# HilaManor/AudioEditingCode

Measured on AMD Instinct MI355X. Metric: edited-clips/sec (200-step inv+edit, 10 s@16 kHz), higher is better.
Workload: dtype f32

## Files before the change

audioeditingcode_amd/_lib.py:

```python
import ctypes
import os

import torch

_HERE = os.path.dirname(os.path.abspath(__file__))
LIB_PATH = os.path.join(_HERE, "libaed.so")


class aed_op(ctypes.Structure):
    _fields_ = [("code", ctypes.c_int32), ("flags", ctypes.c_int32), ("i", ctypes.c_int32 * 40),
                ("f", ctypes.c_float * 8), ("p", ctypes.c_void_p * 10)]


OP_NOP, OP_CONV_GEMM, OP_GN_STATS, OP_GN_APPLY, OP_LAYERNORM, OP_ATTENTION, OP_GEGLU, OP_COPY2D, \
    OP_TIME_EMBED, OP_SOFTMAX_ROWS, OP_TRANSPOSE, OP_AXPBY, OP_INVERT_STEP, OP_REVERSE_STEP, OP_DDIM_STEP, \
    OP_ADVANCE, OP_REFLECT_PAD, OP_MAGNITUDE, OP_NCHW_TO_NHWC, OP_NHWC_TO_NCHW, OP_SPLITK_REDUCE, \
    OP_GN_SCALE_SHIFT, OP_GN_SMALL, OP_XATTN_FOLD, OP_ROTARY, OP_SNAKE, OP_SA_STEP, OP_GAUSS_SAMPLE, \
    OP_REVERSE_STEP_VARIANTS, OP_DRIFT_STEP_VARIANTS, OP_REVERSE_STEP_ROWS = range(31)
OP_NAMES = ["nop", "conv_gemm", "gn_stats", "gn_apply", "layernorm", "attention", "geglu", "copy2d", "time_embed",
            "softmax_rows", "transpose", "axpby", "invert_step", "reverse_step", "ddim_step", "advance",
            "reflect_pad", "magnitude", "nchw_to_nhwc", "nhwc_to_nchw", "splitk_reduce", "gn_scale_shift", "gn_small",
            "xattn_fold", "rotary", "snake", "sa_step", "gauss_sample", "reverse_step_variants",
            "drift_step_variants", "reverse_step_rows"]
OP_PC_PROBE, OP_PC_JACOBIAN, OP_PC_ORTHONORMALISE = 31, 32, 33
# ... 3 lines not shown
T5_ATTN_HEAD_SIZES = (8, 16, 32, 64)
T5_ATTN_MAX_L = 512
OP_LAYERNORM_ROWS, OP_ADD_ROWS, OP_GELU_NEW, OP_CAUSAL_ATTENTION = 41, 42, 43, 44
LM_ATTN_HEAD_SIZES = (8, 16, 32, 64)
LM_ATTN_MAX_NK = 1024
SEG_MAX_P = 8
PC_TAB_STRIDE = 4
PC_MAX_EV = 8
ACT_NONE, ACT_SILU, ACT_LEAKY, ACT_TANH, ACT_LOGCLAMP = range(5)
COEF_STRIDE = 8
SA_COEF_STRIDE = 12

_lib = None


class AedError(RuntimeError):
    pass


def lib():
    global _lib
    if _lib is None:
        if not os.path.exists(LIB_PATH):
            raise AedError(f"{LIB_PATH} is missing: build it with `python __graft_entry__.py` "
                           f"(audioeditingcode_amd/csrc/build.sh). There is no CPU fallback.")
        L = ctypes.CDLL(LIB_PATH)
        vp, ci, cf = ctypes.c_void_p, ctypes.c_int, ctypes.c_float
        L.aed_version.restype = ci
        L.aed_last_error.restype = ctypes.c_char_p
        L.aed_device_info.argtypes = [ctypes.POINTER(ci), ctypes.POINTER(ci), ctypes.c_char_p, ci]
        L.aed_launch.argtypes = [ctypes.POINTER(aed_op), vp]
        L.aed_tape_run.argtypes = [ctypes.POINTER(aed_op), ci, vp]
        L.aed_tape_profile.argtypes = [ctypes.POINTER(aed_op), ci, vp, ctypes.POINTER(cf)]
        L.aed_graph_begin.argtypes = [vp]
        L.aed_graph_end.argtypes = [vp, ctypes.POINTER(vp)]
        L.aed_graph_launch.argtypes = [vp, vp]
        L.aed_graph_destroy.argtypes = [vp]
        L.aed_stream_create_cu_mask.argtypes = [ctypes.POINTER(vp), ctypes.POINTER(ctypes.c_uint32), ci, ci]
        L.aed_stream_destroy.argtypes = [vp]
        L.aed_cu_census.argtypes = [vp, ci, ci, vp]
        u64 = ctypes.c_uint64
        L.aed_image_load.argtypes = [ctypes.c_char_p, ci, ctypes.POINTER(vp)]
        L.aed_image_free.argtypes = [vp]
        L.aed_image_run.argtypes = [vp, ctypes.c_char_p, vp]
        L.aed_image_program.argtypes = [vp, ctypes.c_char_p, ctypes.POINTER(ctypes.POINTER(aed_op)), ctypes.POINTER(ci)]
        L.aed_image_buffer.argtypes = [vp, ctypes.c_char_p, ctypes.POINTER(vp), ctypes.POINTER(u64)]
        L.aed_image_copy_in.argtypes = [vp, ctypes.c_char_p, vp, u64, vp]
        L.aed_image_copy_out.argtypes = [vp, ctypes.c_char_p, vp, u64, vp]
        L.aed_event_create.argtypes = [ctypes.POINTER(vp)]
        L.aed_event_record.argtypes = [vp, vp]
        L.aed_event_elapsed_ms.argtypes = [vp, vp, ctypes.POINTER(cf)]
        L.aed_event_destroy.argtypes = [vp]
        fp = ctypes.POINTER(cf)
        L.aed_get_zs_from_xts.argtypes = [vp, vp, vp, vp, vp, cf, ci, fp, ci, ci, vp, vp, ctypes.c_int64, vp]
        L.aed_reverse_step_with_custom_noise.argtypes = [vp, vp, vp, vp, cf, ci, fp, ci, vp, vp, ctypes.c_int64, vp]
        L.aed_reverse_step_variants.argtypes = [vp, vp, vp, ci, fp, ci, vp, vp, ctypes.c_int64, vp]
        L.aed_reverse_step_clips.argtypes = [vp, vp, vp, ci, fp, ci, vp, vp, ctypes.c_int64, vp]
        L.aed_reverse_step_rows.argtypes = [vp, vp, vp, ci, fp, ci, ctypes.POINTER(vp), vp, ctypes.c_int64, vp]
        L.aed_drift_step_variants.argtypes = [vp, vp, vp, ci, fp, ci, vp, vp, vp, ci, ci, vp, vp, ci, cf, ctypes.c_int64, vp]
        L.aed_sample_xts_from_x0.argtypes = [vp, vp, vp, vp, vp, ci, ctypes.c_int64, vp]
        L.aed_mx_quantize_rows.argtypes = [vp, vp, vp, ctypes.c_longlong, ci, vp]
        L.aed_resample_sinc.argtypes = [vp, ci, ctypes.c_int64, vp, ci, ci, ci, vp, ctypes.c_int64, vp]
        L.aed_sa_get_zs_from_xts.argtypes = [vp, vp, vp, vp, cf, fp, vp, ci, vp, vp, ctypes.c_int64, vp]
        L.aed_sa_reverse_step_with_custom_noise.argtypes = [vp, vp, vp, cf, fp, vp, vp, vp, ctypes.c_int64, vp]
        L.aed_sa_reverse_step_variants.argtypes = [vp, vp, vp, ci, fp, ctypes.POINTER(ci), ci, vp, vp, vp, ctypes.c_int64, vp]
        for name in ("aed_launch", "aed_tape_run", "aed_tape_profile", "aed_graph_begin", "aed_graph_end",
                     "aed_graph_launch", "aed_graph_destroy", "aed_stream_create_cu_mask", "aed_stream_destroy",
                     "aed_cu_census", "aed_image_load", "aed_image_free", "aed_image_run", "aed_image_program",
                     "aed_image_buffer", "aed_image_copy_in", "aed_image_copy_out", "aed_event_create", "aed_event_record", "aed_event_elapsed_ms", "aed_event_destroy", "aed_get_zs_from_xts",
                     "aed_reverse_step_with_custom_noise", "aed_reverse_step_variants", "aed_reverse_step_clips", "aed_reverse_step_rows", "aed_drift_step_variants", "aed_sample_xts_from_x0", "aed_device_info",
                     "aed_sa_get_zs_from_xts", "aed_sa_reverse_step_with_custom_noise", "aed_sa_reverse_step_variants",
                     "aed_mx_quantize_rows", "aed_resample_sinc"):
            getattr(L, name).restype = ci
        if L.aed_version() != 4:
            raise AedError("libaed.so ABI version mismatch")
        _lib = L
    return _lib


EXPORTS = ["aed_version", "aed_last_error", "aed_device_info", "aed_launch", "aed_tape_run", "aed_tape_profile",
           "aed_graph_begin", "aed_graph_end", "aed_graph_launch", "aed_graph_destroy", "aed_stream_create_cu_mask",
           "aed_stream_destroy", "aed_cu_census", "aed_image_load", "aed_image_free", "aed_image_run", "aed_image_program",
           "aed_image_buffer", "aed_image_copy_in", "aed_image_copy_out", "aed_event_create",
           "aed_event_record", "aed_event_elapsed_ms", "aed_event_destroy", "aed_get_zs_from_xts",
           "aed_reverse_step_with_custom_noise", "aed_reverse_step_variants", "aed_reverse_step_clips", "aed_reverse_step_rows", "aed_drift_step_variants", "aed_sample_xts_from_x0",
           "aed_sa_get_zs_from_xts",
           "aed_sa_reverse_step_with_custom_noise", "aed_sa_reverse_step_variants", "aed_mx_quantize_rows", "aed_resample_sinc"]


def check(rc, what=""):
    if rc != 0:
        raise AedError(f"{what} failed (rc={rc}): {lib().aed_last_error().decode()}")


def current_stream_ptr():
    import torch
    return ctypes.c_void_p(torch.cuda.current_stream().cuda_stream)
```

audioeditingcode_amd/csrc/api.hip:

```cpp
#include <stdarg.h>
#include <string.h>
#include <vector>
#include "aed_common.h"

static thread_local char g_err[512] = "";
void aed_set_error(const char* fmt, ...) {
    va_list ap;
    va_start(ap, fmt);
    vsnprintf(g_err, sizeof(g_err), fmt, ap);
    va_end(ap);
}

static int g_cus = 0;
int aed_num_cus() {
    if (g_cus == 0) {
        int dev = 0;
        hipDeviceProp_t prop;
        if (hipGetDevice(&dev) == hipSuccess && hipGetDeviceProperties(&prop, dev) == hipSuccess)
            g_cus = prop.multiProcessorCount;
        if (g_cus <= 0) g_cus = 256;
    }
    return g_cus;
}

__global__ void cu_census_kernel(uint32_t* out, int spin) {
    long long t0 = __builtin_readcyclecounter();
    while (__builtin_readcyclecounter() - t0 < spin) __builtin_amdgcn_s_sleep(8);
    if (threadIdx.x == 0) {
        out[2 * blockIdx.x] = __builtin_amdgcn_s_getreg((4) | (0 << 6) | (31 << 11));
        out[2 * blockIdx.x + 1] = __builtin_amdgcn_s_getreg((20) | (0 << 6) | (31 << 11));
    }
}

typedef int (*launcher_t)(const aed_op*, hipStream_t);
static int launch_nop(const aed_op*, hipStream_t) { return 0; }
static int launch_retired(const aed_op* op, hipStream_t) {
    aed_set_error("opcode %d was retired in ABI v4 (fused into conv_gemm: ln_mode / geglu slots)", op->code);
    return 3;
}
int launch_conv_gemm_x6(const aed_op* op, hipStream_t s);
int launch_conv_gemm_f8(const aed_op* op, hipStream_t s);
static int launch_conv_gemm_any(const aed_op* op, hipStream_t s) {
    if (op->flags & 64) return launch_conv_gemm_f8(op, s);
    return (op->flags & 4) ? launch_conv_gemm_x6(op, s) : launch_conv_gemm(op, s);
}
static launcher_t g_table[AED_OP_COUNT] = {
    launch_nop,
    launch_conv_gemm_any,
    launch_gn_stats, launch_gn_apply, launch_retired, launch_attention, launch_retired, launch_copy2d,
    launch_time_embed, launch_softmax_rows, launch_transpose, launch_axpby, launch_invert_step,
    launch_reverse_step, launch_ddim_step, launch_advance, launch_reflect_pad, launch_magnitude,
    launch_layout, launch_layout, launch_splitk_reduce, launch_gn_scale_shift, launch_gn_small, launch_xattn_fold,
    launch_rotary, launch_snake, launch_sa_step, launch_gauss_sample, launch_reverse_step_variants,
    launch_drift_step_variants, launch_reverse_step_rows, launch_pc_probe, launch_pc_jacobian, launch_pc_orthonormalise,
    launch_sa_step_variants, launch_reverse_step_segments,
    launch_t5_embed, launch_rmsnorm, launch_t5_attention, launch_gated_act,
    nullptr,
    launch_layernorm_rows, launch_add_rows, launch_gelu_new, launch_causal_attention,
};

extern "C" {

int aed_version(void) { return AED_VERSION; }
const char* aed_last_error(void) { return g_err; }

int aed_device_info(int* cu_count, int* lds_bytes, char* arch, int arch_len) {
    int dev = 0;
    hipDeviceProp_t prop;
    AED_CHECK_HIP(hipGetDevice(&dev));
    AED_CHECK_HIP(hipGetDeviceProperties(&prop, dev));
    if (cu_count) *cu_count = prop.multiProcessorCount;
    if (lds_bytes) *lds_bytes = (int)prop.maxSharedMemoryPerMultiProcessor;
    if (arch && arch_len > 0) {
        strncpy(arch, prop.gcnArchName, arch_len - 1);
        arch[arch_len - 1] = 0;
    }
    return 0;
}

int aed_launch(const aed_op* op, void* stream) {
    AED_REQUIRE(op != nullptr, "aed_launch: null op");
    AED_REQUIRE(op->code >= 0 && op->code < AED_OP_COUNT && g_table[op->code] != nullptr, "aed_launch: bad opcode %d", op->code);
    return g_table[op->code](op, (hipStream_t)stream);
}

int aed_tape_run(const aed_op* ops, int n, void* stream) {
    AED_REQUIRE(ops != nullptr || n == 0, "aed_tape_run: null tape");
    for (int k = 0; k < n; ++k) {
        const aed_op* op = ops + k;
        if (op->code < 0 || op->code >= AED_OP_COUNT || g_table[op->code] == nullptr) {
            aed_set_error("aed_tape_run: bad opcode %d at op %d", op->code, k);
            return 2;
        }
        int rc = g_table[op->code](op, (hipStream_t)stream);
        if (rc) {
            char tmp[400];
            strncpy(tmp, g_err, sizeof(tmp) - 1);
            tmp[sizeof(tmp) - 1] = 0;
            aed_set_error("op %d (code %d): %s", k, op->code, tmp);
            return rc;
        }
    }
    return 0;
}

int aed_tape_profile(const aed_op* ops, int n, void* stream, float* ms_host) {
    AED_REQUIRE(ops && ms_host, "aed_tape_profile: null argument");
    std::vector<hipEvent_t> ev(n + 1);
    for (int k = 0; k <= n; ++k) AED_CHECK_HIP(hipEventCreate(&ev[k]));
    AED_CHECK_HIP(hipEventRecord(ev[0], (hipStream_t)stream));
    for (int k = 0; k < n; ++k) {
        int rc = aed_launch(ops + k, stream);
        if (rc) return rc;
        AED_CHECK_HIP(hipEventRecord(ev[k + 1], (hipStream_t)stream));
    }
    AED_CHECK_HIP(hipEventSynchronize(ev[n]));
    for (int k = 0; k < n; ++k) AED_CHECK_HIP(hipEventElapsedTime(&ms_host[k], ev[k], ev[k + 1]));
    for (int k = 0; k <= n; ++k) (void)hipEventDestroy(ev[k]);
    return 0;
}

int aed_graph_begin(void* stream) {
    AED_CHECK_HIP(hipStreamBeginCapture((hipStream_t)stream, hipStreamCaptureModeThreadLocal));
    return 0;
}
int aed_graph_end(void* stream, void** graph_exec_out) {
    hipGraph_t graph = nullptr;
    AED_CHECK_HIP(hipStreamEndCapture((hipStream_t)stream, &graph));
    hipGraphExec_t exec = nullptr;
    hipError_t e = hipGraphInstantiate(&exec, graph, nullptr, nullptr, 0);
    (void)hipGraphDestroy(graph);
    if (e != hipSuccess) {
        aed_set_error("hipGraphInstantiate: %s", hipGetErrorString(e));
        return 1;
    }
    *graph_exec_out = (void*)exec;
// ... 60 lines not shown
```

audioeditingcode_amd/csrc/cg_params.h:

```cpp
#pragma once
#include "aed_common.h"

typedef float f32x16 __attribute__((ext_vector_type(16)));

struct CGParams {
    const float* A;
    const float* W;
    const float* bias;
    float* C;
    const float* res;
    const float* rowvec;
    float* ws;
    long long* dbg;
    const float* A2;
    int diag;
    int gm;
    int M, N, K;
    int lda, ldc, ldr, ld_rv;
    int IH, IW, OH, OW, Cin;
    int KH, KW, stride, pad_h, pad_w, dil_h, dil_w, up;
    int a_bs;
    int vIH, vIW;
    int o_mul, o_add, o_len, out_bs;
    int in_act, out_act, accumulate, ksplit;
// ... 11 lines not shown
    const float* kbias;
    int geglu;
    const unsigned char* Wq;
    const unsigned char* Wsc;
};

__device__ __forceinline__ float in_transform(float v, int act, float slope) {
    if (act == AED_ACT_SILU) return v / (1.0f + __expf(-v));
    if (act == AED_ACT_LEAKY) return v > 0.0f ? v : v * slope;
    return v;
}

__device__ __forceinline__ float gelu_exact(float g) { return 0.5f * g * (1.0f + erff(g * 0.70710678118654752440f)); }
__device__ __forceinline__ float glu_gate(float g, int kind) { return kind == 2 ? g / (1.0f + expf(-g)) : gelu_exact(g); }

__device__ __forceinline__ void store_out(const CGParams& p, int m, int n, float v) {
    int b = m / p.rpb;
    int q = m - b * p.rpb;
    int o = q * p.o_mul + p.o_add;
    if ((unsigned)o >= (unsigned)p.o_len) return;
    size_t row = (size_t)b * p.out_bs + o;
    if (p.bias) v += p.bias[n];
    if (p.rowvec && !p.ln_mode) v += p.rowvec[(size_t)b * p.ld_rv + n];
    if (p.res) v += p.res[row * p.ldr + n];
    v = aed_apply_act(v, p.out_act, p.out_p);
    float* dst = p.C + row * p.ldc + n;
    if (p.accumulate == 1) v += *dst;
    else if (p.accumulate == 2) v = (*dst + v) / p.out_div;
    *dst = v;
}

int cg_fill_params(const aed_op* op, CGParams& p, int bkt);
int launch_lin_gemm(const CGParams& p, int cfg, hipStream_t s);
```

audioeditingcode_amd/csrc/conv_gemm.hip:

```cpp
#include "cg_params.h"

template <int BM, int BN, int WROWS, int WCOLS, bool GENERIC, int DEPTH, int BKT, bool PLAIN>
__global__ __launch_bounds__(256, (BM * BN >= 128 * 128) ? 2 : 1) void conv_gemm_kernel(CGParams p) {
    constexpr int WM = BM / WROWS, WN = BN / WCOLS;
    constexpr int TM = WM / 32, TN = WN / 32;
    constexpr int LDS_LD = BKT + 4;
    constexpr int STAGE = (BM + BN) * LDS_LD;
    constexpr int TPR = BKT / 4;
    constexpr int RPP = 256 / TPR;
    constexpr int PA = BM / RPP, PB = BN / RPP;
    constexpr int NKB = BKT / 8;
    static_assert(WROWS * WCOLS == 4, "4 waves");
    static_assert(TM >= 1 && TN >= 1 && PA >= 1 && PB >= 1, "tile");

    __shared__ __attribute__((aligned(16))) float lds[2 * STAGE];

    const int tid = threadIdx.x;
    const int lane = tid & 63;
    const int wave = tid >> 6;
    const int wr = wave / WCOLS, wc = wave % WCOLS;
    int tile_x = blockIdx.x, tile_y = blockIdx.y;
    if (gridDim.z == 1) {
        const unsigned nx = gridDim.x, nwg = nx * gridDim.y;
        const unsigned orig = blockIdx.y * nx + blockIdx.x;
// ... 356 lines not shown
                "conv_gemm: operand exceeds the 32-bit element-offset range");
    if (p.ksplit < 1) p.ksplit = 1;
    if (p.ksplit > p.nchunks) p.ksplit = p.nchunks;
    if (p.ksplit > 1) AED_REQUIRE(p.ws != nullptr, "conv_gemm: split-K needs a workspace");
    if (p.ln_mode)
        AED_REQUIRE(p.ksplit == 1 && p.KH * p.KW == 1 && p.rowvec && p.bias && p.in_act == 0,
                    "conv_gemm: fused LayerNorm needs a 1-tap, unsplit GEMM with folded weights");
    if (p.C1 > 0)
        AED_REQUIRE(p.A2 && p.C1 % 64 == 0 && p.C1 < p.Cin && p.lda2 % 4 == 0 && ((uintptr_t)p.A2 % 16) == 0 &&
                        (long long)(p.M / p.rpb) * p.a_bs2 + (long long)p.IH * p.IW * p.lda2 < (1LL << 31),
                    "conv_gemm: bad two-source split C1=%d of Cin=%d", p.C1, p.Cin);
    if (p.geglu)
        AED_REQUIRE(p.ksplit == 1 && p.N % 64 == 0 && !p.res && p.out_act == 0 && p.accumulate == 0 && p.o_mul == 1 &&
                        p.o_add == 0 && p.o_len >= p.rpb && (p.ln_mode || !p.rowvec),
                    "conv_gemm: the GEGLU epilogue needs an unsplit GEMM with packed N %% 64 == 0 and a plain epilogue");
    return 0;
}

template <int BM, int BN, int WR, int WC, int DEPTH, int BKT>
static void launch_cfg(const CGParams& p, bool plain, hipStream_t s) {
    dim3 grid(aed_cdiv(p.N, BN), aed_cdiv(p.M, BM), p.ksplit);
    if (plain)
        hipLaunchKernelGGL((conv_gemm_kernel<BM, BN, WR, WC, false, DEPTH, BKT, true>), grid, dim3(256), 0, s, p);
    else
        hipLaunchKernelGGL((conv_gemm_kernel<BM, BN, WR, WC, false, DEPTH, BKT, false>), grid, dim3(256), 0, s, p);
}

template <int BM, int BN, int WR, int WC>
static void launch_generic(const CGParams& p, hipStream_t s) {
    dim3 grid(aed_cdiv(p.N, BN), aed_cdiv(p.M, BM), p.ksplit);
    hipLaunchKernelGGL((conv_gemm_kernel<BM, BN, WR, WC, true, 1, 32, false>), grid, dim3(256), 0, s, p);
}

int launch_conv_gemm(const aed_op* op, hipStream_t s) {
    CGParams p;
    const int32_t* i = op->i;
    const int Cin = i[11];
    const bool generic = (Cin % 32 != 0) || (i[3] % 4 != 0) || ((uintptr_t)op->p[0] % 16 != 0) ||
                         ((uintptr_t)op->p[1] % 16 != 0);
    int cfg = i[29];
    if (cfg >= 10) {
        int rc = cg_fill_params(op, p, 32);
        if (rc) return rc;
        return launch_lin_gemm(p, cfg, s);
    }
    if (cfg == 0) {
        const int cus = aed_num_cus();
        const int M = i[0], N = i[1], ks = i[28] > 1 ? i[28] : 1;
        auto blocks = [&](int bm, int bn) { return (long)aed_cdiv(M, bm) * aed_cdiv(N, bn) * ks; };
        if (N <= 32) cfg = 5;
        else if (M <= 32) cfg = 6;
        else if (blocks(128, 128) >= (long)cus && N >= 128) cfg = 1;
        else if (blocks(128, 64) >= 2L * cus && N >= 64) cfg = 2;
        else cfg = 4;
        if (N < 64 && cfg != 5) cfg = 5;
    }
    if (generic && (cfg == 1 || cfg == 2 || cfg == 3)) cfg = 4;
    const bool bk64 = !generic && (Cin % 64 == 0) && i[30] != 1 && cfg == 4;
    int rc = cg_fill_params(op, p, bk64 ? 64 : 32);
    if (rc) return rc;
    const bool plain = p.in_act == 0 && p.ln_mode == 0;
    AED_REQUIRE(p.sm_group == 0 && p.w_bs == 0 && p.vec_bs == 0 && p.vec_ld == 1,
                "conv_gemm: per-batch weights / grouped softmax exist only in the lin_gemm kernels (tile >= 10)");
    if (p.geglu) AED_REQUIRE(cfg == 1 || cfg == 3, "conv_gemm: the GEGLU epilogue needs 64-wide wave tiles: 128x128 or 64x128 (cfg %d)", cfg);
    if (p.C1 > 0) AED_REQUIRE(!generic, "conv_gemm: two-source A needs the vector path of a tiled kernel");
    switch (cfg) {
        case 1: launch_cfg<128, 128, 2, 2, 2, 32>(p, plain, s); break;
        case 2: launch_cfg<128, 64, 2, 2, 2, 32>(p, plain, s); break;
        case 3: launch_cfg<64, 128, 2, 2, 2, 32>(p, plain, s); break;
        case 4:
            if (generic) launch_generic<64, 64, 2, 2>(p, s);
            else if (bk64) launch_cfg<64, 64, 2, 2, 2, 64>(p, plain, s);
            else launch_cfg<64, 64, 2, 2, 3, 32>(p, plain, s);
            break;
        case 5:
            if (generic) launch_generic<128, 32, 4, 1>(p, s);
            else launch_cfg<128, 32, 4, 1, 3, 32>(p, plain, s);
            break;
        case 6:
            if (generic) launch_generic<32, 128, 1, 4>(p, s);
            else launch_cfg<32, 128, 1, 4, 3, 32>(p, plain, s);
            break;
        default: AED_REQUIRE(false, "conv_gemm: bad tile cfg %d", cfg);
    }
    AED_CHECK_HIP(hipGetLastError());
    if (p.ksplit > 1) {
        size_t total = (size_t)p.M * p.N;
        int grid = (int)((((p.N & 3) == 0 ? total >> 2 : total) + 255) / 256);
        if (grid > 2048) grid = 2048;
        hipLaunchKernelGGL(splitk_reduce_kernel, dim3(grid), dim3(256), 0, s, p);
        AED_CHECK_HIP(hipGetLastError());
    }
    return 0;
}

int launch_splitk_reduce_slices(const aed_op* op, int slices, hipStream_t s) {
    CGParams p;
    int rc = cg_fill_params(op, p, 32);
    if (rc) return rc;
    if (slices > 0) p.ksplit = slices;
    size_t total = (size_t)p.M * p.N;
    int grid = (int)((((p.N & 3) == 0 ? total >> 2 : total) + 255) / 256);
    if (grid > 2048) grid = 2048;
    hipLaunchKernelGGL(splitk_reduce_kernel, dim3(grid), dim3(256), 0, s, p);
    AED_CHECK_HIP(hipGetLastError());
    return 0;
}

int launch_splitk_reduce(const aed_op* op, hipStream_t s) { return launch_splitk_reduce_slices(op, 0, s); }
```

audioeditingcode_amd/csrc/conv_gemm_x6.hip:

```cpp
#include "cg_params.h"

typedef __bf16 bf16x8 __attribute__((ext_vector_type(8)));
typedef __bf16 bf16x2 __attribute__((ext_vector_type(2)));
typedef float f32x2 __attribute__((ext_vector_type(2)));

int launch_conv_gemm_x6(const aed_op* op, hipStream_t s);

constexpr int X6_BK = 16;

__device__ __forceinline__ void x6_split_pair(float x0, float x1, unsigned& h, unsigned& m, unsigned& l) {
    h = __builtin_bit_cast(unsigned, __builtin_convertvector((f32x2){x0, x1}, bf16x2));
    float r0 = x0 - __uint_as_float(h << 16);
    float r1 = x1 - __uint_as_float(h & 0xffff0000u);
    asm volatile("" : "+v"(r0), "+v"(r1));
    m = __builtin_bit_cast(unsigned, __builtin_convertvector((f32x2){r0, r1}, bf16x2));
    float q0 = r0 - __uint_as_float(m << 16);
    float q1 = r1 - __uint_as_float(m & 0xffff0000u);
    asm volatile("" : "+v"(q0), "+v"(q1));
    l = __builtin_bit_cast(unsigned, __builtin_convertvector((f32x2){q0, q1}, bf16x2));
}

typedef unsigned u32x4 __attribute__((ext_vector_type(4)));
constexpr unsigned X6_OOB = 0x80000000u;

// ... 253 lines not shown
            if constexpr (KB == 2) {
                bf16x8 af2[TM][3], bw2[TN][3];
                load_frags(lds + cur * STAGE, 1, af2, bw2);
                do_mfmas(af2, bw2);
            }
            hints();
            __syncthreads();
            cur ^= 1;
        }
    }

    float* ln_stat = reinterpret_cast<float*>(lds);
#include "cg_epilogue.h"
}

template <int BM, int BN, int WR, int WC, int DEPTH, bool DIAG, int BK = X6_BK>
static int x6_launch(const CGParams& p, bool plain, int sched, int terms, hipStream_t s) {
    dim3 grid(aed_cdiv(p.N, BN), aed_cdiv(p.M, BM), p.ksplit);
    dim3 block(64 * WR * WC);
#define X6_GO(PL, SC, NT_) hipLaunchKernelGGL((conv_gemm_x6_kernel<BM, BN, WR, WC, DEPTH, PL, SC, NT_, BK>), grid, block, 0, s, p)
    if (terms == 3) {
        if constexpr (DIAG) {
            if (plain) { X6_GO(true, 1, 3); return 0; }
        }
        AED_REQUIRE(false, "conv_gemm_x6: the three-term diagnostic exists for tiles 1 and 8 with a plain A operand");
    }
    if (!plain) X6_GO(false, 1, 6);
    else if (sched) X6_GO(true, 1, 6);
    else X6_GO(true, 0, 6);
#undef X6_GO
    return 0;
}

int launch_conv_gemm_x6(const aed_op* op, hipStream_t s) {
    const int32_t* i = op->i;
    const int Cin = i[11];
    int cfg = i[29];
    const long long batch = i[0] / (i[9] * i[10] > 0 ? i[9] * i[10] : 1);
    const bool fits = (Cin % X6_BK == 0) && (i[3] % 4 == 0) && ((uintptr_t)op->p[0] % 16 == 0) &&
                      ((uintptr_t)op->p[1] % 16 == 0) && cfg < 10 && cfg != 5 && cfg != 6 && cfg != 7 && i[36] == 0 &&
                      i[37] == 0 && i[38] <= 1 && i[39] == 0 &&
                      batch * i[20] + (long long)i[7] * i[8] * i[3] < (1LL << 29) && (long long)i[1] * i[2] < (1LL << 29) &&
                      (i[32] == 0 || batch * i[34] + (long long)i[7] * i[8] * i[33] < (1LL << 29));
    if (!fits) {
        if (cfg == 8 || cfg == 9) {
            aed_op fp32_op = *op;
            fp32_op.i[29] = 1;
            return launch_conv_gemm(&fp32_op, s);
        }
        return launch_conv_gemm(op, s);
    }
    const bool wide = (op->flags & 256) && (cfg == 8 || cfg == 9) && Cin % 32 == 0 && !(op->flags & 16);
    CGParams p;
    int rc = cg_fill_params(op, p, wide ? 32 : X6_BK);
    if (rc) return rc;
    if (p.ksplit > (p.K + 31) / 32) p.ksplit = (p.K + 31) / 32;
    if (cfg == 0) {
        const int cus = aed_num_cus();
        auto blocks = [&](int bm, int bn) { return (long)aed_cdiv(p.M, bm) * aed_cdiv(p.N, bn) * p.ksplit; };
        if (p.N >= 512 && p.N % 256 == 0 && blocks(128, 256) >= 2L * cus) cfg = 9;
        else if (blocks(256, 128) >= 2L * cus && p.N >= 128) cfg = 8;
        else if (blocks(128, 128) >= (long)cus && p.N >= 128) cfg = 1;
        else if (blocks(128, 64) >= 2L * cus) cfg = 2;
        else cfg = 4;
    }
    if (!(op->flags & 1024) && p.ksplit <= 1) {
        static const int BMs[10] = {0, 128, 128, 64, 64, 0, 0, 0, 256, 128}, BNs[10] = {0, 128, 64, 128, 64, 0, 0, 0, 128, 256};
        const int nx = aed_cdiv(p.N, BNs[cfg]), ny = aed_cdiv(p.M, BMs[cfg]);
        const int resident = ((aed_num_cus() >> ((op->flags >> 16) & 3)) / 8) * ((cfg == 8 || cfg == 9) ? 1 : 2);
        if (nx > 1 && ny > 1) {
            int g = 1;
            while (g * 2 <= ny && (long)(g * 2) * (g * 2) * BMs[cfg] <= (long)resident * BNs[cfg]) g *= 2;
            if (resident / g < nx) p.gm = g;
            if (op->flags & 0x3800) p.gm = 1 << ((op->flags >> 11) & 7);
        }
    }
    const bool plain = p.in_act == 0 && p.ln_mode == 0;
    const int sched = (op->flags & 8) ? 1 : 0;
    const int terms = (op->flags & 16) ? 3 : 6;
    if (p.geglu) AED_REQUIRE(cfg == 1 || cfg == 3 || cfg == 8 || cfg == 9, "conv_gemm_x6: the GEGLU epilogue needs 64-wide wave tiles (cfg %d)", cfg);
    switch (cfg) {
        case 1: rc = x6_launch<128, 128, 2, 2, 2, true>(p, plain, sched, terms, s); break;
        case 2: rc = x6_launch<128, 64, 2, 2, 2, false>(p, plain, sched, terms, s); break;
        case 3: rc = x6_launch<64, 128, 2, 2, 2, false>(p, plain, sched, terms, s); break;
        case 4: rc = x6_launch<64, 64, 2, 2, 2, false>(p, plain, sched, terms, s); break;
        case 8: rc = wide && terms == 6 ? x6_launch<256, 128, 4, 2, 2, false, 32>(p, plain, sched, terms, s)
                                        : x6_launch<256, 128, 4, 2, 2, true>(p, plain, sched, terms, s); break;
        case 9: rc = wide && terms == 6 ? x6_launch<128, 256, 2, 4, 2, false, 32>(p, plain, sched, terms, s)
                                        : x6_launch<128, 256, 2, 4, 2, false>(p, plain, sched, terms, s); break;
        default: AED_REQUIRE(false, "conv_gemm_x6: bad tile cfg %d", cfg);
    }
    if (rc) return rc;
    AED_CHECK_HIP(hipGetLastError());
    if (p.ksplit > 1) return launch_splitk_reduce(op, s);
    return 0;
}
```

audioeditingcode_amd/csrc/norm.hip:

```cpp
#include "aed_common.h"

__device__ __forceinline__ const float* gn_src(const float* x, const float* x2, int C1, int ldx, int ldx2, size_t row,
                                               int c) {
    return (x2 != nullptr && c >= C1) ? x2 + row * ldx2 + (c - C1) : x + row * ldx + c;
}

__device__ __forceinline__ float gn_shift(const float4& v) { return 0.25f * ((v.x + v.y) + (v.z + v.w)); }

__device__ __forceinline__ void gn_acc(const float4& v, float k, float& s, float& ss) {
    const float a = v.x - k, b = v.y - k, c = v.z - k, d = v.w - k;
    s += (a + b) + (c + d);
    ss += fmaf(a, a, b * b) + fmaf(c, c, d * d);
}

__device__ __forceinline__ void gn_rebase(float s, float ss, float k, int n, double& S, double& SS) {
    const double dk = (double)k, ds = (double)s, dn = (double)n;
    S = ds + dn * dk;
    SS = (double)ss + dk * (2.0 * ds + dn * dk);
}

struct gn_moments { float mean_hi, mean_lo, rstd; double mean; };
__device__ __forceinline__ gn_moments gn_block_moments(double ds, double dss, double* rs, double* rss, double n, float eps) {
    const int tid = threadIdx.x;
#pragma unroll
    for (int o = 32; o > 0; o >>= 1) { ds += __shfl_xor(ds, o, 64); dss += __shfl_xor(dss, o, 64); }
    if ((tid & 63) == 0) { rs[tid >> 6] = ds; rss[tid >> 6] = dss; }
    __syncthreads();
    ds = (rs[0] + rs[1]) + (rs[2] + rs[3]);
    dss = (rss[0] + rss[1]) + (rss[2] + rss[3]);
    gn_moments m;
    m.mean = ds / n;
    double var = dss / n - m.mean * m.mean;
    if (var < 0.0) var = 0.0;
// ... 274 lines not shown
    gn_rebase(s, ss, k, tid < total ? (total - tid + 255) / 256 : 0, ds, dss);
    const gn_moments m = gn_block_moments(ds, dss, rs, rss, (double)HW * (double)cpg, eps);
    for (int e = tid; e < total; e += 256) {
        const int row = e / cpg, c = g * cpg + (e - row * cpg);
        y[(rb + row) * ldy + c] = gn_out(*src(e), m.mean_hi, m.mean_lo, m.rstd, gamma[c], beta[c], act);
    }
}

int launch_gn_small(const aed_op* op, hipStream_t s) {
    const int32_t* i = op->i;
    AED_REQUIRE(op->p[0] && op->p[1] && op->p[2] && op->p[3], "gn_small: null pointer");
    AED_REQUIRE(i[3] > 0 && i[2] % i[3] == 0, "gn_small: C=%d G=%d", i[2], i[3]);
    AED_REQUIRE(!op->p[4] || (i[8] > 0 && i[8] < i[2]), "gn_small: bad two-source split");
    if (i[2] % (4 * i[3]) != 0 || i[4] % 4 != 0 || i[5] % 4 != 0 || (op->p[4] && (i[8] % 4 != 0 || i[9] % 4 != 0))) {
        hipLaunchKernelGGL(gn_generic_kernel, dim3(i[3], i[0]), dim3(256), 0, s, (const float*)op->p[0], (const float*)op->p[1],
                           (const float*)op->p[2], (float*)op->p[3], i[1], i[2], i[3], i[4], i[5], op->f[0], i[6],
                           (const float*)op->p[4], i[8], i[9]);
        AED_CHECK_HIP(hipGetLastError());
        return 0;
    }
    const int total4 = i[1] * (i[2] / i[3] / 4);
#define GN_ARGS (const float*)op->p[0], (const float*)op->p[1], (const float*)op->p[2], (float*)op->p[3], i[1], i[2], i[3], \
                i[4], i[5], op->f[0], i[6], (const float*)op->p[4], i[8], i[9]
    const dim3 grid(i[3], i[0]);
    if (i[7] != 1 && total4 <= 256 * 2) hipLaunchKernelGGL(gn_small_reg_kernel<2>, grid, dim3(256), 0, s, GN_ARGS);
    else if (i[7] != 1 && total4 <= 256 * 4) hipLaunchKernelGGL(gn_small_reg_kernel<4>, grid, dim3(256), 0, s, GN_ARGS);
    else if (i[7] != 1 && total4 <= 256 * 8) hipLaunchKernelGGL(gn_small_reg_kernel<8>, grid, dim3(256), 0, s, GN_ARGS);
    else hipLaunchKernelGGL(gn_small_kernel<4>, grid, dim3(256), 0, s, GN_ARGS);
#undef GN_ARGS
    AED_CHECK_HIP(hipGetLastError());
    return 0;
}

int launch_gn_scale_shift(const aed_op* op, hipStream_t s) {
    const int32_t* i = op->i;
    AED_REQUIRE(op->p[0] && op->p[1] && op->p[2] && op->p[3], "gn_scale_shift: null pointer");
    AED_REQUIRE(i[2] % (4 * i[3]) == 0 && i[2] / i[3] <= 256 && i[4] % 4 == 0, "gn_scale_shift: C=%d G=%d", i[2], i[3]);
    hipLaunchKernelGGL(gn_scale_shift_kernel, dim3(i[3], i[0]), dim3(256), 0, s, (const float*)op->p[0],
                       (const float*)op->p[1], (const float*)op->p[2], (float*)op->p[3], i[1], i[2], i[3], i[4],
                       op->f[0]);
    AED_CHECK_HIP(hipGetLastError());
    return 0;
}

int launch_gn_stats(const aed_op* op, hipStream_t s) {
    const int32_t* i = op->i;
    AED_REQUIRE(op->p[0] && op->p[1], "gn_stats: null pointer");
    AED_REQUIRE(i[3] <= 64 && i[2] % (4 * i[3]) == 0, "gn_stats: C=%d must be a multiple of 4*G (G=%d<=64)", i[2], i[3]);
    AED_REQUIRE(i[4] % 4 == 0, "gn_stats: ldx %% 4");
    AED_REQUIRE(i[5] > 0 && i[6] > 0 && (int64_t)(i[6] - 1) * i[5] < i[1], "gn_stats: %d chunks of %d rows over HW=%d", i[6], i[5],
                i[1]);
    hipLaunchKernelGGL(gn_stats_kernel, dim3(i[6], i[0]), dim3(256), 0, s, (const float*)op->p[0], (float*)op->p[1],
                       i[1], i[2], i[3], i[4], i[5], i[6], (const float*)op->p[2], i[7], i[8]);
    AED_CHECK_HIP(hipGetLastError());
    return 0;
}

int launch_gn_apply(const aed_op* op, hipStream_t s) {
    const int32_t* i = op->i;
    AED_REQUIRE(op->p[0] && op->p[1] && op->p[2] && op->p[3] && op->p[4], "gn_apply: null pointer");
    AED_REQUIRE(i[3] <= 64 && 256 % i[3] == 0 && i[2] % (4 * i[3]) == 0, "gn_apply: C=%d G=%d", i[2], i[3]);
    AED_REQUIRE(i[12] > 0 && i[6] > 0 && (int64_t)(i[6] - 1) * i[12] < i[1] && (int64_t)i[6] * i[12] >= i[1],
                "gn_apply: %d partials of %d rows do not tile HW=%d", i[6], i[12], i[1]);
    hipLaunchKernelGGL(gn_apply_kernel, dim3(i[9], i[0]), dim3(256), 0, s, (const float*)op->p[0],
                       (const float*)op->p[1], (const float*)op->p[2], (const float*)op->p[3], (float*)op->p[4], i[1],
                       i[2], i[3], i[4], i[8], i[5], i[6], op->f[0], i[7], (const float*)op->p[5], i[10], i[11], i[12]);
// ... 5 lines not shown
```

include/aed.h:

```cpp
#ifndef AED_H
#define AED_H
#include <stdint.h>

#ifdef __cplusplus
extern "C" {
#endif

#define AED_VERSION 4

enum aed_opcode {
    AED_OP_NOP = 0,
    AED_OP_CONV_GEMM = 1,
    AED_OP_GN_STATS = 2,
    AED_OP_GN_APPLY = 3,
    AED_OP_LAYERNORM = 4,
    AED_OP_ATTENTION = 5,
    AED_OP_GEGLU = 6,
    AED_OP_COPY2D = 7,
    AED_OP_TIME_EMBED = 8,
    AED_OP_SOFTMAX_ROWS = 9,
    AED_OP_TRANSPOSE = 10,
    AED_OP_AXPBY = 11,
    AED_OP_INVERT_STEP = 12,
    AED_OP_REVERSE_STEP = 13,
// ... 17 lines not shown
    AED_OP_PC_PROBE = 31,
    AED_OP_PC_JACOBIAN = 32,
    AED_OP_PC_ORTHONORMALISE = 33,
    AED_OP_SA_STEP_VARIANTS = 34,
    AED_OP_REVERSE_STEP_SEGMENTS = 35,
    AED_OP_T5_EMBED = 36,
    AED_OP_RMSNORM = 37,
    AED_OP_T5_ATTENTION = 38,
    AED_OP_GATED_ACT = 39,
    AED_OP_LAYERNORM_ROWS = 41,
    AED_OP_ADD_ROWS = 42,
    AED_OP_GELU_NEW = 43,
    AED_OP_CAUSAL_ATTENTION = 44,
    AED_OP_COUNT
};

typedef struct aed_op {
    int32_t code;
    int32_t flags;
    int32_t i[40];
    float   f[8];
    void*   p[10];
} aed_op;

enum aed_act { AED_ACT_NONE = 0, AED_ACT_SILU = 1, AED_ACT_LEAKY = 2, AED_ACT_TANH = 3, AED_ACT_LOGCLAMP = 4 };

int         aed_version(void);
const char* aed_last_error(void);
int         aed_device_info(int* cu_count, int* lds_bytes, char* arch, int arch_len);

int aed_launch(const aed_op* op, void* stream);
int aed_tape_run(const aed_op* ops, int n, void* stream);
int aed_tape_profile(const aed_op* ops, int n, void* stream, float* ms_host);

int aed_graph_begin(void* stream);
int aed_graph_end(void* stream, void** graph_exec_out);
int aed_graph_launch(void* graph_exec, void* stream);
int aed_graph_destroy(void* graph_exec);

int aed_stream_create_cu_mask(void** stream_out, const uint32_t* mask_words, int n_words, int priority);
int aed_stream_destroy(void* stream);
int aed_cu_census(uint32_t* out_dev, int n_blocks, int spin_clocks, void* stream);

int aed_image_load(const char* path, int flags, void** image_out);
int aed_image_free(void* image);
int aed_image_run(void* image, const char* program, void* stream);
int aed_image_program(void* image, const char* program, const aed_op** ops_out, int* n_out);
int aed_image_buffer(void* image, const char* name, void** ptr_out, uint64_t* nbytes_out);
int aed_image_copy_in(void* image, const char* name, const void* host, uint64_t nbytes, void* stream);
int aed_image_copy_out(void* image, const char* name, void* host, uint64_t nbytes, void* stream);

int aed_event_create(void** ev_out);
int aed_event_record(void* ev, void* stream);
int aed_event_elapsed_ms(void* ev_start, void* ev_stop, float* ms_out);
int aed_event_destroy(void* ev);


#define AED_COEF_STRIDE 8

int aed_get_zs_from_xts(const float* xt, float* xtm1, const float* eps_u, const float* eps_c,
                        const float* cfg, float cfg_scalar, int n_prompts, const float* coef_host,
                        int v_prediction, int numerical_fix, float* z, float* noise_pred_out,
                        int64_t numel, void* stream);

int aed_reverse_step_with_custom_noise(const float* xt, const float* eps_u, const float* eps_c,
                                       const float* cfg, float cfg_scalar, int n_prompts,
// ... 47 lines not shown
```

Baseline: 0.9830.

## Fuse split-K GEMM reduction with following GroupNorm in tape runner

Adds a tape planner that detects a conv_gemm with split-K followed by a small GroupNorm reading its output. It launches the GEMM slabs only and then one kernel that reduces the split-K partials, applies bias, residual and activation, writes C, and computes the GroupNorm output in the same pass. This removes the separate splitk_reduce kernel and the re-read of C by GroupNorm. The cost is a per-op planning check with alias tests, and a single workgroup per group that may leave parallelism unused. It is enabled by default through the AED_TAPE_FUSION environment variable, with a size bound.

New measurement: 0.9851, median of 6. About the same (+0.2%).

```diff
diff --git a/audioeditingcode_amd/_lib.py b/audioeditingcode_amd/_lib.py
--- a/audioeditingcode_amd/_lib.py
+++ b/audioeditingcode_amd/_lib.py
@@ -59,6 +59,10 @@
         L.aed_launch.argtypes = [ctypes.POINTER(aed_op), vp]
         L.aed_tape_run.argtypes = [ctypes.POINTER(aed_op), ci, vp]
         L.aed_tape_profile.argtypes = [ctypes.POINTER(aed_op), ci, vp, ctypes.POINTER(cf)]
+        L.aed_tape_plan.argtypes = [ctypes.POINTER(aed_op), ci, ctypes.POINTER(ci)]
+        L.aed_tape_plan.restype = ci
+        L.aed_tape_set_fusion.argtypes = [ci]
+        L.aed_tape_set_fusion.restype = ci
         L.aed_graph_begin.argtypes = [vp]
         L.aed_graph_end.argtypes = [vp, ctypes.POINTER(vp)]
         L.aed_graph_launch.argtypes = [vp, vp]
@@ -106,6 +110,7 @@
 
 
 EXPORTS = ["aed_version", "aed_last_error", "aed_device_info", "aed_launch", "aed_tape_run", "aed_tape_profile",
+           "aed_tape_plan", "aed_tape_set_fusion",
            "aed_graph_begin", "aed_graph_end", "aed_graph_launch", "aed_graph_destroy", "aed_stream_create_cu_mask",
            "aed_stream_destroy", "aed_cu_census", "aed_image_load", "aed_image_free", "aed_image_run", "aed_image_program",
            "aed_image_buffer", "aed_image_copy_in", "aed_image_copy_out", "aed_event_create",
diff --git a/audioeditingcode_amd/csrc/api.hip b/audioeditingcode_amd/csrc/api.hip
--- a/audioeditingcode_amd/csrc/api.hip
+++ b/audioeditingcode_amd/csrc/api.hip
@@ -1,7 +1,10 @@
 #include <stdarg.h>
+#include <stdlib.h>
 #include <string.h>
 #include <vector>
 #include "aed_common.h"
+#include "cg_params.h"
+#include "tape_plan.h"
 
 static thread_local char g_err[512] = "";
 void aed_set_error(const char* fmt, ...) {
@@ -59,6 +62,24 @@
     launch_layernorm_rows, launch_add_rows, launch_gelu_new, launch_causal_attention,
 };
 
+static int g_fusion = -1;
+static int fusion_mode() {
+    if (g_fusion < 0) {
+        const char* e = getenv("AED_TAPE_FUSION");
+        const int v = e ? atoi(e) : 1;
+        g_fusion = v < 0 ? 0 : (v > 2 ? 2 : v);
+    }
+    return g_fusion;
+}
+static long long fusion_bound(int mode) { return mode == 2 ? 0 : (long long)AED_SPLITK_GN_MAX_BYTES; }
+
+static int launch_fused_pair(const aed_op* gemm, const aed_op* gn, hipStream_t s) {
+    CGParams p;
+    int rc = (gemm->flags & 4) ? launch_conv_gemm_x6_slabs(gemm, s, &p) : launch_conv_gemm_slabs(gemm, s, &p);
+    if (rc) return rc;
+    return p.ksplit > 1 ? launch_splitk_gn(p, gn, s) : launch_gn_small(gn, s);
+}
+
 extern "C" {
 
 int aed_version(void) { return AED_VERSION; }
@@ -86,13 +107,23 @@
 
 int aed_tape_run(const aed_op* ops, int n, void* stream) {
     AED_REQUIRE(ops != nullptr || n == 0, "aed_tape_run: null tape");
+    const int mode = fusion_mode();
     for (int k = 0; k < n; ++k) {
         const aed_op* op = ops + k;
         if (op->code < 0 || op->code >= AED_OP_COUNT || g_table[op->code] == nullptr) {
             aed_set_error("aed_tape_run: bad opcode %d at op %d", op->code, k);
             return 2;
         }
-        int rc = g_table[op->code](op, (hipStream_t)stream);
+        int rc;
+        if (mode && k + 1 < n && aed_plan_pair(op, op + 1, fusion_bound(mode))) {
+            rc = launch_fused_pair(op, op + 1, (hipStream_t)stream);
+            if (!rc) {
+                ++k;
+                continue;
+            }
+        } else {
+            rc = g_table[op->code](op, (hipStream_t)stream);
+        }
         if (rc) {
             char tmp[400];
             strncpy(tmp, g_err, sizeof(tmp) - 1);
@@ -102,6 +133,17 @@
         }
     }
     return 0;
+}
+
+int aed_tape_plan(const aed_op* ops, int n, int* fused_at) {
+    AED_REQUIRE(ops != nullptr || n == 0, "aed_tape_plan: null tape");
+    const int mode = fusion_mode();
+    return mode ? aed_plan_tape(ops, n, fused_at, fusion_bound(mode)) : 0;
+}
+int aed_tape_set_fusion(int mode) {
+    const int prev = fusion_mode();
+    g_fusion = mode < 0 ? 0 : (mode > 2 ? 2 : mode);
+    return prev;
 }
 
 int aed_tape_profile(const aed_op* ops, int n, void* stream, float* ms_host) {
diff --git a/audioeditingcode_amd/csrc/cg_params.h b/audioeditingcode_amd/csrc/cg_params.h
--- a/audioeditingcode_amd/csrc/cg_params.h
+++ b/audioeditingcode_amd/csrc/cg_params.h
@@ -67,3 +67,6 @@
 
 int cg_fill_params(const aed_op* op, CGParams& p, int bkt);
 int launch_lin_gemm(const CGParams& p, int cfg, hipStream_t s);
+int launch_conv_gemm_slabs(const aed_op* op, hipStream_t s, CGParams* p);
+int launch_conv_gemm_x6_slabs(const aed_op* op, hipStream_t s, CGParams* p);
+int launch_splitk_gn(const CGParams& p, const aed_op* gn, hipStream_t s);
diff --git a/audioeditingcode_amd/csrc/conv_gemm.hip b/audioeditingcode_amd/csrc/conv_gemm.hip
--- a/audioeditingcode_amd/csrc/conv_gemm.hip
+++ b/audioeditingcode_amd/csrc/conv_gemm.hip
@@ -412,7 +412,7 @@
     hipLaunchKernelGGL((conv_gemm_kernel<BM, BN, WR, WC, true, 1, 32, false>), grid, dim3(256), 0, s, p);
 }
 
-int launch_conv_gemm(const aed_op* op, hipStream_t s) {
+static int conv_gemm_impl(const aed_op* op, hipStream_t s, CGParams* slabs) {
     CGParams p;
     const int32_t* i = op->i;
     const int Cin = i[11];
@@ -422,6 +422,7 @@
     if (cfg >= 10) {
         int rc = cg_fill_params(op, p, 32);
         if (rc) return rc;
+        if (slabs) *slabs = p;
         return launch_lin_gemm(p, cfg, s);
     }
     if (cfg == 0) {
@@ -464,6 +465,10 @@
         default: AED_REQUIRE(false, "conv_gemm: bad tile cfg %d", cfg);
     }
     AED_CHECK_HIP(hipGetLastError());
+    if (slabs) {
+        *slabs = p;
+        return 0;
+    }
     if (p.ksplit > 1) {
         size_t total = (size_t)p.M * p.N;
         int grid = (int)((((p.N & 3) == 0 ? total >> 2 : total) + 255) / 256);
@@ -473,6 +478,9 @@
     }
     return 0;
 }
+
+int launch_conv_gemm(const aed_op* op, hipStream_t s) { return conv_gemm_impl(op, s, nullptr); }
+int launch_conv_gemm_slabs(const aed_op* op, hipStream_t s, CGParams* p) { return conv_gemm_impl(op, s, p); }
 
 int launch_splitk_reduce_slices(const aed_op* op, int slices, hipStream_t s) {
     CGParams p;
diff --git a/audioeditingcode_amd/csrc/conv_gemm_x6.hip b/audioeditingcode_amd/csrc/conv_gemm_x6.hip
--- a/audioeditingcode_amd/csrc/conv_gemm_x6.hip
+++ b/audioeditingcode_amd/csrc/conv_gemm_x6.hip
@@ -309,7 +309,7 @@
     return 0;
 }
 
-int launch_conv_gemm_x6(const aed_op* op, hipStream_t s) {
+static int conv_gemm_x6_impl(const aed_op* op, hipStream_t s, CGParams* slabs) {
     const int32_t* i = op->i;
     const int Cin = i[11];
     int cfg = i[29];
@@ -323,9 +323,9 @@
         if (cfg == 8 || cfg == 9) {
             aed_op fp32_op = *op;
             fp32_op.i[29] = 1;
-            return launch_conv_gemm(&fp32_op, s);
-        }
-        return launch_conv_gemm(op, s);
+            return slabs ? launch_conv_gemm_slabs(&fp32_op, s, slabs) : launch_conv_gemm(&fp32_op, s);
+        }
+        return slabs ? launch_conv_gemm_slabs(op, s, slabs) : launch_conv_gemm(op, s);
     }
     const bool wide = (op->flags & 256) && (cfg == 8 || cfg == 9) && Cin % 32 == 0 && !(op->flags & 16);
     CGParams p;
@@ -369,6 +369,13 @@
     }
     if (rc) return rc;
     AED_CHECK_HIP(hipGetLastError());
+    if (slabs) {
+        *slabs = p;
+        return 0;
+    }
     if (p.ksplit > 1) return launch_splitk_reduce(op, s);
     return 0;
 }
+
+int launch_conv_gemm_x6(const aed_op* op, hipStream_t s) { return conv_gemm_x6_impl(op, s, nullptr); }
+int launch_conv_gemm_x6_slabs(const aed_op* op, hipStream_t s, CGParams* p) { return conv_gemm_x6_impl(op, s, p); }
diff --git a/audioeditingcode_amd/csrc/norm.hip b/audioeditingcode_amd/csrc/norm.hip
--- a/audioeditingcode_amd/csrc/norm.hip
+++ b/audioeditingcode_amd/csrc/norm.hip
@@ -1,4 +1,5 @@
 #include "aed_common.h"
+#include "cg_params.h"
 
 __device__ __forceinline__ const float* gn_src(const float* x, const float* x2, int C1, int ldx, int ldx2, size_t row,
                                                int c) {
@@ -339,6 +340,146 @@
     return 0;
 }
 
+struct SGParams {
+    const float* ws; const float* bias; const float* rowvec; const float* res; float* C;
+    int M, N, ksplit, ldc, ldr, ld_rv, rpb, out_act;
+    float out_p;
+    const float* gamma; const float* beta; float* y; const float* x2;
+    int HW, Cg, G, ldy, C1, ldx2, act;
+    float eps;
+};
+
+template <int U, int ZB>
+__global__ __launch_bounds__(256) void splitk_gn_kernel(SGParams p) {
+    __shared__ double rs[4], rss[4];
+    const int tid = threadIdx.x, b = blockIdx.y;
+    const int bx = blockIdx.x;
+    const int g = (p.G & 7) == 0 ? (bx & 7) * (p.G >> 3) + (bx >> 3) : bx;
+    const int cpg = p.Cg / p.G, cpg4 = cpg >> 2;
+    const size_t rb = (size_t)b * p.HW;
+    float* yb = p.y + (size_t)b * p.HW * p.ldy + g * cpg;
+    const int total = p.HW * cpg4;
+    const size_t q4 = ((size_t)p.M * p.N) >> 2;
+    float4 v[U], ga[U], be[U];
+    int rowv[U], jv[U];
+    bool own[U];
+    const float4* src[U];
+#pragma unroll
+    for (int u = 0; u < U; ++u) {
+        const int e = min(tid + 256 * u, total - 1);
+        rowv[u] = e / cpg4;
+        jv[u] = e - rowv[u] * cpg4;
+        const int c = g * cpg + 4 * jv[u];
+        own[u] = !(p.x2 != nullptr && c >= p.C1);
+        src[u] = own[u] ? reinterpret_cast<const float4*>(p.ws) + (((rb + rowv[u]) * p.N + c) >> 2)
+                        : reinterpret_cast<const float4*>(p.x2 + (rb + rowv[u]) * p.ldx2 + (c - p.C1));
+    }
+    const bool has_b = p.bias != nullptr, has_rv = p.rowvec != nullptr, has_r = p.res != nullptr;
+    float bi[U][4], rw[U][4], rsd[U][4];
+    bool fin[U];
+#pragma unroll
+    for (int u = 0; u < U; ++u) {
+        v[u] = *src[u];
+        ga[u] = *reinterpret_cast<const float4*>(p.gamma + g * cpg + 4 * jv[u]);
+        be[u] = *reinterpret_cast<const float4*>(p.beta + g * cpg + 4 * jv[u]);
+        fin[u] = own[u] && tid + 256 * u < total;
+        const int n = own[u] ? g * cpg + 4 * jv[u] : 0;
+        const unsigned m = (unsigned)(rb + rowv[u]);
+        const float* any = p.ws;
+        const float* bp = has_b ? p.bias + n : any;
+        const float* rvp = has_rv ? p.rowvec + (size_t)(m / (unsigned)p.rpb) * p.ld_rv + n : any;
+        const float* rsp = (has_r && fin[u]) ? p.res + (size_t)m * p.ldr + n : any;
+#pragma unroll
+        for (int j = 0; j < 4; ++j) {
+            bi[u][j] = bp[j];
+            rw[u][j] = rvp[j];
+            rsd[u][j] = rsp[j];
+        }
+    }
+    auto round = [&](int z0) {
+        float4 w[ZB][U];
+#pragma unroll
+        for (int zz = 0; zz < ZB; ++zz) {
+            const size_t zo = (size_t)min(z0 + zz, p.ksplit - 1) * q4;
+#pragma unroll
+            for (int u = 0; u < U; ++u) w[zz][u] = src[u][own[u] ? zo : 0];
+        }
+        __builtin_amdgcn_sched_barrier(0);
+#pragma unroll
+        for (int zz = 0; zz < ZB; ++zz) {
+            const bool on = z0 + zz < p.ksplit;
+#pragma unroll
+            for (int u = 0; u < U; ++u) {
+                if (!(on && own[u])) continue;
+                v[u].x += w[zz][u].x; v[u].y += w[zz][u].y; v[u].z += w[zz][u].z; v[u].w += w[zz][u].w;
+            }
+        }
+    };
+    round(1);
+    for (int z0 = 1 + ZB; z0 < p.ksplit; z0 += ZB) round(z0);
+#pragma unroll
+    for (int u = 0; u < U; ++u) {
+        if (!fin[u]) continue;
+        float o[4] = {v[u].x, v[u].y, v[u].z, v[u].w};
+#pragma unroll
+        for (int j = 0; j < 4; ++j) {
+            if (has_b) o[j] += bi[u][j];
+            if (has_rv) o[j] += rw[u][j];
+            if (has_r) o[j] += rsd[u][j];
+            o[j] = aed_apply_act(o[j], p.out_act, p.out_p);
+        }
+        v[u] = make_float4(o[0], o[1], o[2], o[3]);
+        *reinterpret_cast<float4*>(p.C + (rb + rowv[u]) * p.ldc + g * cpg + 4 * jv[u]) = v[u];
+    }
+    float s = 0.f, ss = 0.f;
+    const float k = tid < total ? gn_shift(v[0]) : 0.f;
+#pragma unroll
+    for (int u = 0; u < U; ++u) {
+        if (tid + 256 * u < total) gn_acc(v[u], k, s, ss);
+    }
+    double ds, dss;
+    gn_rebase(s, ss, k, tid < total ? 4 * ((total - tid + 255) / 256) : 0, ds, dss);
+    const gn_moments m = gn_block_moments(ds, dss, rs, rss, (double)p.HW * (double)cpg, p.eps);
+#pragma unroll
+    for (int u = 0; u < U; ++u) {
+        if (tid + 256 * u >= total) continue;
+        *reinterpret_cast<float4*>(yb + (size_t)rowv[u] * p.ldy + 4 * jv[u]) =
+            gn_out4(v[u], m.mean_hi, m.mean_lo, m.rstd, ga[u], be[u], p.act);
+    }
+}
+
+int launch_splitk_gn(const CGParams& p, const aed_op* gn, hipStream_t s) {
+    const int32_t* i = gn->i;
+    const int cpg = i[3] > 0 ? i[2] / i[3] : 0;
+    const int total4 = i[1] * (cpg / 4);
+    AED_REQUIRE(p.ksplit > 1 && p.ws && (p.N & 3) == 0 && (p.ldc & 3) == 0, "splitk_gn: not a float4 split-K site");
+    AED_REQUIRE(gn->p[0] == (void*)p.C && i[4] == p.ldc && i[0] > 0 && (long long)i[0] * i[1] == p.M,
+                "splitk_gn: the GroupNorm does not read the GEMM's rows");
+    AED_REQUIRE(cpg > 0 && cpg % 4 == 0 && i[2] == cpg * i[3] && i[5] % 4 == 0 && total4 > 0 && total4 <= 256 * 8,
+                "splitk_gn: C=%d G=%d HW=%d", i[2], i[3], i[1]);
+    AED_REQUIRE(gn->p[4] ? (i[8] == p.N && i[8] < i[2] && i[9] % 4 == 0) : i[2] == p.N, "splitk_gn: columns of C not covered once");
+    SGParams q;
+    q.ws = p.ws; q.bias = p.bias; q.rowvec = p.rowvec; q.res = p.res; q.C = p.C;
+    q.M = p.M; q.N = p.N; q.ksplit = p.ksplit; q.ldc = p.ldc; q.ldr = p.ldr; q.ld_rv = p.ld_rv; q.rpb = p.rpb; q.out_act = p.out_act;
+    q.out_p = p.out_p;
+    q.gamma = (const float*)gn->p[1]; q.beta = (const float*)gn->p[2]; q.y = (float*)gn->p[3]; q.x2 = (const float*)gn->p[4];
+    q.HW = i[1]; q.Cg = i[2]; q.G = i[3]; q.ldy = i[5]; q.C1 = i[8]; q.ldx2 = i[9]; q.act = i[6];
+    q.eps = gn->f[0];
+    const dim3 grid(i[3], i[0]);
+    const int need = p.ksplit - 1;
+#define SG_LAUNCH(U_, ZB_) hipLaunchKernelGGL((splitk_gn_kernel<U_, ZB_>), grid, dim3(256), 0, s, q)
+    if (total4 <= 256 * 2) {
+        if (need <= 1) SG_LAUNCH(2, 1); else if (need <= 3) SG_LAUNCH(2, 3); else if (need <= 7) SG_LAUNCH(2, 7); else SG_LAUNCH(2, 15);
+    } else if (total4 <= 256 * 4) {
+        if (need <= 1) SG_LAUNCH(4, 1); else if (need <= 3) SG_LAUNCH(4, 3); else SG_LAUNCH(4, 7);
+    } else {
+        if (need <= 1) SG_LAUNCH(8, 1); else if (need <= 3) SG_LAUNCH(8, 3); else SG_LAUNCH(8, 4);
+    }
+#undef SG_LAUNCH
+    AED_CHECK_HIP(hipGetLastError());
+    return 0;
+}
+
 int launch_gn_scale_shift(const aed_op* op, hipStream_t s) {
     const int32_t* i = op->i;
     AED_REQUIRE(op->p[0] && op->p[1] && op->p[2] && op->p[3], "gn_scale_shift: null pointer");
diff --git a/audioeditingcode_amd/csrc/tape_plan.h b/audioeditingcode_amd/csrc/tape_plan.h
--- /dev/null
+++ b/audioeditingcode_amd/csrc/tape_plan.h
@@ -0,0 +1,75 @@
+#pragma once
+#include <stdint.h>
+#include "../../include/aed.h"
+
+#define AED_SPLITK_GN_MAX_BYTES (128 * 1024)
+#define AED_SPLITK_GN_MIN_WGS 64
+
+#define AED_SPLITK_GN_MAX_SLICE4 (256 * 8)
+
+static inline bool aed_plan_overlap(const void* a, long long na, const void* b, long long nb) {
+    if (!a || !b || na <= 0 || nb <= 0) return false;
+    const uintptr_t a0 = (uintptr_t)a, b0 = (uintptr_t)b;
+    return a0 < b0 + (uintptr_t)nb && b0 < a0 + (uintptr_t)na;
+}
+
+static inline int aed_plan_ksplit(const aed_op* g) {
+    const int chunks = (g->i[2] + 31) / 32;
+    return g->i[28] < chunks ? g->i[28] : chunks;
+}
+
+static inline bool aed_plan_pair(const aed_op* g, const aed_op* n, long long max_bytes) {
+    if (g->code != AED_OP_CONV_GEMM || n->code != AED_OP_GN_SMALL) return false;
+    const int32_t* gi = g->i;
+    const int32_t* ni = n->i;
+    if (g->flags & (64 | 0x8000)) return false;
+    if (gi[29] >= 10 || gi[29] == 7) return false;
+    const int M = gi[0], N = gi[1], K = gi[2], ldc = gi[4], rpb = gi[9] * gi[10];
+    if (M <= 0 || N <= 0 || K <= 64 || rpb <= 0) return false;
+    if (gi[28] <= 1 || g->p[6] == nullptr || g->p[3] == nullptr) return false;
+    if (!(gi[21] == 1 && gi[22] == 0 && gi[24] == rpb && gi[23] == rpb && gi[27] == 0)) return false;
+    if (N % 4 != 0 || ldc % 4 != 0 || ((uintptr_t)g->p[3] % 16) != 0 || ((uintptr_t)g->p[6] % 16) != 0) return false;
+    if (gi[31] != 0 || gi[35] != 0) return false;
+    if (gi[26] == AED_ACT_LEAKY) return false;
+    const int B = ni[0], HW = ni[1], C = ni[2], G = ni[3], ldy = ni[5];
+    if (n->p[0] != g->p[3] || ni[4] != ldc) return false;
+    if (!n->p[1] || !n->p[2] || !n->p[3]) return false;
+    if (B <= 0 || HW <= 0 || (long long)B * HW != M || M % rpb != 0) return false;
+    if (G <= 0 || C % G != 0 || (C / G) % 4 != 0 || ldy % 4 != 0) return false;
+    if (ni[7] == 1) return false;
+    const long long slice4 = (long long)HW * (C / G / 4);
+    if (slice4 > AED_SPLITK_GN_MAX_SLICE4) return false;
+    if (n->p[4]) {
+        if (ni[8] != N || ni[8] >= C || ni[9] % 4 != 0 || ((uintptr_t)n->p[4] % 16) != 0) return false;
+    } else if (C != N) {
+        return false;
+    }
+    const long long c_bytes = ((long long)(M - 1) * ldc + N) * 4, ws_bytes = (long long)gi[28] * M * N * 4;
+    const long long y_bytes = ((long long)(M - 1) * ldy + C) * 4;
+    const long long batch = M / rpb;
+    const void* y = n->p[3];
+    if (aed_plan_overlap(y, y_bytes, g->p[3], c_bytes) || aed_plan_overlap(y, y_bytes, g->p[6], ws_bytes)) return false;
+    if (aed_plan_overlap(y, y_bytes, g->p[2], (long long)N * 4) ||
+        aed_plan_overlap(y, y_bytes, g->p[5], ((batch - 1) * gi[6] + N) * 4) ||
+        aed_plan_overlap(y, y_bytes, g->p[4], ((long long)(M - 1) * gi[5] + N) * 4))
+        return false;
+    if (g->p[4] && g->p[4] != g->p[3] && aed_plan_overlap(g->p[4], ((long long)(M - 1) * gi[5] + N) * 4, g->p[3], c_bytes))
+        return false;
+    if (g->p[4] == g->p[3] && gi[5] != ldc) return false;
+    if (aed_plan_overlap(n->p[1], (long long)C * 4, g->p[3], c_bytes) || aed_plan_overlap(n->p[2], (long long)C * 4, g->p[3], c_bytes))
+        return false;
+    if (n->p[4] && aed_plan_overlap(n->p[4], ((long long)(M - 1) * ni[9] + (C - N)) * 4, g->p[3], c_bytes)) return false;
+    if (max_bytes > 0 && ((long long)aed_plan_ksplit(g) * slice4 * 16 > max_bytes || (long long)B * G < AED_SPLITK_GN_MIN_WGS)) return false;
+    return true;
+}
+
+static inline int aed_plan_tape(const aed_op* ops, int n, int* fused_at, long long max_bytes) {
+    int pairs = 0;
+    for (int k = 0; k + 1 < n; ++k) {
+        if (!aed_plan_pair(ops + k, ops + k + 1, max_bytes)) continue;
+        if (fused_at) fused_at[pairs] = k;
+        ++pairs;
+        ++k;
+    }
+    return pairs;
+}
diff --git a/include/aed.h b/include/aed.h
--- a/include/aed.h
+++ b/include/aed.h
@@ -73,6 +73,8 @@
 int aed_launch(const aed_op* op, void* stream);
 int aed_tape_run(const aed_op* ops, int n, void* stream);
 int aed_tape_profile(const aed_op* ops, int n, void* stream, float* ms_host);
+int aed_tape_plan(const aed_op* ops, int n, int* fused_at);
+int aed_tape_set_fusion(int mode);
 
 int aed_graph_begin(void* stream);
 int aed_graph_end(void* stream, void** graph_exec_out);
```
